# gwall-ceres/HighRes-net

Measured on AMD Instinct MI355X. Metric: SR frames/sec (384x384 out) at B=32, n_views=32, higher is better.
Workload: dtype bf16

## Files before the change

highres-net_amd/hrnet_hip/csrc/conv3x3_v6_impl.h:

```cpp
#pragma once
#include <type_traits>
#include "conv3x3.h"

#ifndef V6_ABL
#define V6_ABL 0
#endif
#ifndef V6_ST_AUX
#define V6_ST_AUX 2
#endif
#ifndef V6_RES_NT
#define V6_RES_NT 1
#endif
#ifndef V6_BAL
#define V6_BAL 4
#endif

#ifdef V6_STAMP
extern __device__ unsigned long long hrn_v6_stamps[256 * 8 * 24];
#define V6_ST(i) do { unsigned long long t_; asm volatile("s_memtime %0\n\ts_waitcnt lgkmcnt(0)" : "=s"(t_) :: "memory"); if (stamp_on) st[i] = t_; } while (0)
#else
#define V6_ST(i) do {} while (0)
#endif

namespace {

constexpr int T6_H = 16, T6_W = 32;
constexpr int HW6 = T6_W + 2;
constexpr int NPIX6 = (T6_H + 2) * HW6;
constexpr int N_IN6 = (NPIX6 * 64 + 1023) / 1024;
constexpr int IN_BYTES6 = N_IN6 * 1024;
constexpr unsigned OOB6 = 0x80000000u;

template <int COUT, bool X3 = false> struct G6 {
    static constexpr int NCB = COUT / 16;
    static constexpr int NQ = NCB / 2;
    static constexpr int TAP_BYTES = COUT * 64;
    static constexpr int WST = 3 * TAP_BYTES;
    static constexpr int W_PIECES = WST / 1024;
    static constexpr int OFF_IN = 2 * WST;
    static constexpr int OFF_BIAS = OFF_IN + 2 * IN_BYTES6;
    static constexpr int ROW = COUT * 2;
    static constexpr int LB = NCB * 2;
    static constexpr int OFF_FIFO = OFF_BIAS + 512;
    static constexpr int FIFO_WAVE = (LB == 16 && !X3) ? 4096 : 0;
    static constexpr int OFF_HOFF = OFF_FIFO + 8 * FIFO_WAVE;
    static constexpr int LDS_BYTES = OFF_HOFF + (X3 ? 8 * 5 * 256 : 0);
};

typedef __attribute__((address_space(3))) void* lds_ptr6;

template <int N> __device__ __forceinline__ void wait_vm6() {
    static_assert(N >= 0 && N <= 63, "vmcnt");
    asm volatile("s_waitcnt vmcnt(%0)" :: "n"(N) : "memory");
}
__device__ __forceinline__ void wait_vm6_rt(int n) {
    switch (n) {
        case 1: wait_vm6<1>(); break;
        case 2: wait_vm6<2>(); break;
        case 3: wait_vm6<3>(); break;
        case 4: wait_vm6<4>(); break;
        case 5: wait_vm6<5>(); break;
        case 6: wait_vm6<6>(); break;
        case 7: wait_vm6<7>(); break;
        case 8: wait_vm6<8>(); break;
        case 9: wait_vm6<9>(); break;
        default: wait_vm6<0>(); break;
    }
}
__device__ __forceinline__ void barrier6() {
    asm volatile("s_waitcnt lgkmcnt(0)" ::: "memory");
    __builtin_amdgcn_s_barrier();
    asm volatile("" ::: "memory");
}
__device__ __forceinline__ int swz6(int row) { return ((row >> 2) & 1) << 1; }

template <int N, int I = 0, class F> __device__ __forceinline__ void static_for6(F&& f) {
    if constexpr (I < N) { f(std::integral_constant<int, I>{}); static_for6<N, I + 1>(f); }
}

template <int CIN, int COUT, int RESM, bool PAIR, bool X3>
__global__ __launch_bounds__(512, 2) void conv3x3_v6_kernel(const ConvParams p) {
    typedef G6<COUT, X3> GEO;
    static_assert(CIN == 128 || (CIN == 64 && !PAIR), "CIN");
    constexpr int NCH = CIN / 32;
    constexpr int NCC = X3 ? 3 * NCH : NCH;
    constexpr int NCB = GEO::NCB, NQ = GEO::NQ, NSTEP = 3 * NQ, WST = GEO::WST, TAP_BYTES = GEO::TAP_BYTES;
    constexpr int OFF_IN = GEO::OFF_IN, ROW = GEO::ROW, LB = GEO::LB;
    typedef typename std::conditional<LB == 16, u32x4, u32x2>::type lane_row_t;
    constexpr bool RES = RESM != 0;
    constexpr int BAL = COUT == 128 ? V6_BAL : 0;
    extern __shared__ __attribute__((aligned(16))) unsigned char smem[];
    float* bias_lds = (float*)(smem + GEO::OFF_BIAS);
    if (p.only_if_nonpos && p.only_if_nonpos[0] > 0.f) return;

    const int tid = threadIdx.x;
    const int lane = tid & 63;
    const int w = __builtin_amdgcn_readfirstlane(tid >> 6);
    const int c15 = lane & 15, q = lane >> 4;
    const int H = p.H, W = p.W;
    const unsigned hw = (unsigned)(H * W);
    const unsigned tiles_x = (W + T6_W - 1) / T6_W;
    const unsigned tiles_y = (H + T6_H - 1) / T6_H;
    const unsigned tiles = tiles_x * tiles_y;
    const unsigned total = tiles * (unsigned)p.M;
    const unsigned G = gridDim.x;
    const unsigned bid = blockIdx.x;
    const unsigned slot0 = (G & 7) == 0 ? (bid & 7) * (G >> 3) + (bid >> 3) : bid;
    if (slot0 >= total) return;
    const int ntl = (int)((total - slot0 + G - 1) / G);
    unsigned cur_m = slot0 / tiles, cur_t = slot0 - cur_m * tiles;
    const unsigned step_m = G / tiles, step_t = G - step_m * tiles;
    constexpr bool in_pair = PAIR;
    constexpr unsigned in_pitch = in_pair ? 128u : (unsigned)(CIN * 2);
    const size_t src_lo = X3 ? (in_pair ? p.stack_lo : p.in_lo) : 0;
    const unsigned char* const src0 = (const unsigned char*)(in_pair ? p.stack : p.in);
    const unsigned img_bytes = hw * in_pitch;

    auto in_bases = [&](unsigned m, size_t& a, size_t& b) __attribute__((always_inline)) {
        if (in_pair) {
            const unsigned bb = m / (unsigned)p.pair_h, i = m - bb * (unsigned)p.pair_h;
            a = ((size_t)bb * p.pair_vs + i) * hw * 128;
            b = ((size_t)bb * p.pair_vs + (p.pair_last - i)) * hw * 128;
        } else {
            a = b = (size_t)m * hw * in_pitch;
        }
    };
    unsigned hoff[5];
    auto tile_offsets = [&](unsigned t) __attribute__((always_inline)) {
        const int ty = t / tiles_x;
        const int y0 = ty * T6_H, x0 = (t - ty * tiles_x) * T6_W;
        int lq = lane;
        asm volatile("" : "+v"(lq));
#pragma unroll
        for (int jj = 0; jj < 5; ++jj) {
            const int pix = (w + 8 * jj) * 16 + (lq >> 2);
            const int lc = (lq & 3) ^ swz6(pix);
            const int py = pix / HW6, px = pix - py * HW6;
            const int gy = y0 - 1 + py, gx = x0 - 1 + px;
            const bool ok = pix < NPIX6 && (unsigned)gy < (unsigned)H && (unsigned)gx < (unsigned)W;
            const unsigned ho = ok ? (unsigned)(gy * W + gx) * in_pitch + (unsigned)(lc * 16) : OOB6;
            if constexpr (X3) *(unsigned*)(smem + GEO::OFF_HOFF + (w * 5 + jj) * 256 + lq * 4) = ho;
            else hoff[jj] = ho;
        }
    };
    auto dma_halo_v = [&](__amdgpu_buffer_rsrc_t rs, int c, int buf, int jj, unsigned voff) __attribute__((always_inline)) {
        const int j = w + 8 * jj;
        if (j < N_IN6) {
            const unsigned soff = in_pair ? (unsigned)((c & 1) * 64) : (unsigned)(c * 64);
            if (!(V6_ABL & 4)) __builtin_amdgcn_raw_ptr_buffer_load_lds(rs, (lds_ptr6)(smem + OFF_IN + buf * IN_BYTES6 + j * 1024), 16, voff, soff, 0, 0);
        }
    };
    auto hoff_lds = [&](int jj) __attribute__((always_inline)) -> unsigned {
        return *(const unsigned*)(smem + GEO::OFF_HOFF + (w * 5 + jj) * 256 + lane * 4);
    };
    auto dma_halo = [&](__amdgpu_buffer_rsrc_t rs, int c, int buf, int jj) __attribute__((always_inline)) {
        if constexpr (X3) dma_halo_v(rs, c, buf, jj, hoff_lds(jj));
        else dma_halo_v(rs, c, buf, jj, hoff[jj]);
    };
    constexpr unsigned W_PLANE = 9u * CIN * COUT * 2u;
    const __amdgpu_buffer_rsrc_t rs_w = __builtin_amdgcn_make_buffer_rsrc((void*)p.wpk, 0, (int)(W_PLANE * (X3 ? 2 : 1)), 0x00020000);
    const unsigned w_lane_off = (unsigned)((lane >> 2) * (NCB * 128) + (((lane & 3) ^ swz6(lane >> 2)) << 4));
    auto dma_w = [&](int c, int tg, int slot_, int t3, unsigned plane_off) __attribute__((always_inline)) {
        const int qq = w + 8 * t3;
        if (qq < GEO::W_PIECES) {
            const int kx = qq / NCB, jb = qq - kx * NCB;
            const unsigned soff = plane_off + (unsigned)(((c >> 1) * 9 + tg * 3 + kx) * (COUT * 128) + (c & 1) * 64 + jb * 128);
            if (!(V6_ABL & 4)) __builtin_amdgcn_raw_ptr_buffer_load_lds(rs_w, (lds_ptr6)(smem + slot_ * WST + kx * TAP_BYTES + jb * 1024), 16, w_lane_off, soff, 0, 0);
        }
    };
    constexpr int NW3 = (GEO::W_PIECES + 7) / 8;
    const int n_in = w < (N_IN6 & 7) ? (N_IN6 >> 3) + 1 : (N_IN6 >> 3);

    const float act_slope = p.slope ? p.slope[0] : 1.f;
    const float act_pick = act_slope <= 1.f ? __builtin_inff() : -__builtin_inff();

    const unsigned lds0 = (unsigned)(__UINTPTR_TYPE__)(__attribute__((address_space(3))) unsigned char*)smem;
    const unsigned a_off = lds0 + (unsigned)(c15 * 64 + ((q ^ swz6(c15)) << 4));
    unsigned baddr[4][3];
#pragma unroll
    for (int j = 0; j < 4; ++j)
#pragma unroll
        for (int kx = 0; kx < 3; ++kx) {
            const int pix = (2 * w + j) * HW6 + c15 + kx;
            baddr[j][kx] = lds0 + (unsigned)OFF_IN + (unsigned)(pix << 6) + ((unsigned)(q << 4) ^ (unsigned)((pix & 4) << 3));
        }

    f32x4 acc[NCB][4];
#ifdef V6_STAMP
    unsigned long long st[24];
#pragma unroll
    for (int i = 0; i < 24; ++i) st[i] = 0;
    bool stamp_on = false;
#endif

    if (tid < COUT) bias_lds[tid] = p.bias[tid];
    size_t inA, inB;
    in_bases(cur_m, inA, inB);
    tile_offsets(cur_t);
    {
        const __amdgpu_buffer_rsrc_t rs = __builtin_amdgcn_make_buffer_rsrc((void*)(src0 + inA), 0, (int)img_bytes, 0x00020000);
#pragma unroll
        for (int t3 = 0; t3 < NW3; ++t3) dma_w(0, 0, 0, t3, 0u);
#pragma unroll
        for (int jj = 0; jj < 5; ++jj) dma_halo(rs, 0, 0, jj);
    }
    wait_vm6<0>();
    barrier6();

    for (int tl = 0; tl < ntl; ++tl) {
        const bool more_tiles = tl + 1 < ntl;
#ifdef V6_STAMP
        stamp_on = false;
        if (RESM == 2 && !PAIR && ntl >= 32 && tl == 1) { stamp_on = true; V6_ST(20); }
        if (RESM == 2 && !PAIR && ntl >= 32 && tl == 2) { stamp_on = true; V6_ST(21); stamp_on = false; }
#endif
        unsigned nxt_t = cur_t + step_t, nxt_m = cur_m + step_m;
        if (nxt_t >= tiles) { nxt_t -= tiles; ++nxt_m; }
        size_t nxA = inA, nxB = inB;
        if (more_tiles) in_bases(nxt_m, nxA, nxB);
#pragma unroll
        for (int cb4 = 0; cb4 < NCB; cb4 += 4) {
            const f32x4 b = *(const f32x4*)(bias_lds + NCB * c15 + cb4);
#pragma unroll
            for (int e = 0; e < 4; ++e)
#pragma unroll
                for (int pxb = 0; pxb < 4; ++pxb) acc[cb4 + e][pxb] = f32x4{b[e], b[e], b[e], b[e]};
        }
        const int ty_ = cur_t / tiles_x;
        const int y0 = ty_ * T6_H, x0 = (cur_t - ty_ * tiles_x) * T6_W;
        const unsigned char *resA = nullptr, *resB = nullptr;
        unsigned char* outp;
        float res_alpha = 1.f;
        {
            size_t oimg = cur_m;
            if (p.out_h > 0) {
                const unsigned ob = cur_m / (unsigned)p.out_h, oi = cur_m - ob * (unsigned)p.out_h;
                oimg = (size_t)ob * p.out_vs + oi;
                if (RESM == 3) {
                    resA = resB = (const unsigned char*)p.res + ((size_t)ob * p.res_vs + oi) * hw * 128;
                    if (p.alphas) res_alpha = p.alphas[(size_t)ob * p.alpha_vs + (p.pair_last - oi)];
                }
            }
            if (RESM == 2) {
                const unsigned bb = cur_m / (unsigned)p.pair_h, i = cur_m - bb * (unsigned)p.pair_h;
                resA = (const unsigned char*)p.stack + ((size_t)bb * p.pair_vs + i) * hw * 128;
                resB = (const unsigned char*)p.stack + ((size_t)bb * p.pair_vs + (p.pair_last - i)) * hw * 128;
            }
            if (RESM == 1) resA = resB = (const unsigned char*)p.res + (size_t)cur_m * hw * ROW;
            outp = (unsigned char*)p.out + oimg * hw * ROW;
        }
        auto res_src = [&](int r, int j) __attribute__((always_inline)) -> const unsigned char* {
            int lq = lane;
            asm volatile("" : "+v"(lq));
            const int c15r = lq & 15, qr = lq >> 4;
            const int gy = y0 + 2 * w + (r >> 1), gyc = gy < H ? gy : H - 1;
            const int gx = x0 + 16 * (r & 1) + 4 * qr + j, gxc = gx < W ? gx : W - 1;
            const unsigned char* view = (RESM == 2 && c15r >= 8) ? resB : resA;
            constexpr int RPITCH = RESM == 1 ? ROW : 128;
            if (V6_ABL & 64) return resA + ((unsigned)(((gyc * W + gxc) & 511) * RPITCH) + (RESM == 2 ? (unsigned)((c15r & 7) * 16) : (unsigned)(c15r * LB)));
            return view + ((unsigned)((gyc * W + gxc) * RPITCH) + (RESM == 2 ? (unsigned)((c15r & 7) * 16) : (unsigned)(c15r * LB)));
        };
        constexpr bool FIFO = RES && LB == 16 && !X3;
        auto res_dma0 = [&]() __attribute__((always_inline)) {
#pragma unroll
            for (int j = 0; j < 4; ++j)
                if (!(V6_ABL & 16))
                    __builtin_amdgcn_global_load_lds((const __attribute__((address_space(1))) void*)res_src(0, j),
                                                     (lds_ptr6)(smem + GEO::OFF_FIFO + w * GEO::FIFO_WAVE + j * 1024), 16, 0, V6_RES_NT ? 2 : 0);
        };

        int c = 0, ps = 0;
        for (int cc = 0; cc < NCC; ++cc) {
            if ((cc > 0 || tl > 0) && (!X3 || ps != 1)) {
                const unsigned d = (X3 ? ps == 2 : (c & 1) != 0) ? (unsigned)IN_BYTES6 : (unsigned)-IN_BYTES6;
#pragma unroll
                for (int j = 0; j < 4; ++j)
#pragma unroll
                    for (int kx = 0; kx < 3; ++kx) baddr[j][kx] += d;
            }
            if (cc == NCC - 1) {
                inA = nxA; inB = nxB;
                if (more_tiles) tile_offsets(nxt_t);
            }
            auto stage = [&](auto tg_c) __attribute__((always_inline)) {
                constexpr int tg = decltype(tg_c)::value;
#ifdef V6_STAMP
                const bool so_ = stamp_on;
                stamp_on = so_ && (cc == 1 || (cc == NCC - 1 && tg == 2));
                const int sb_ = cc == 1 ? 4 * tg : 12;
                V6_ST(sb_ + 0);
#endif
                const int slot_r = (cc + tg) & 1;
                const bool have_next = cc < NCC - 1 || tg < 2 || more_tiles;
                const bool next_chunk = (!X3 || ps != 1) && (cc < NCC - 1 || more_tiles);
                const int tg2 = (tg + 1) % 3;
                int c2 = c;
                unsigned wpl2 = 0;
                if (X3) {
                    int ps2 = ps;
                    if (tg == 2) { if (++ps2 == 3) { ps2 = 0; c2 = (c + 1) & (NCH - 1); } }
                    wpl2 = ps2 == 1 ? W_PLANE : 0u;
                } else {
                    c2 = (c + (tg + 1) / 3) & (NCH - 1);
                }
                const bool nlo = X3 && ps == 0;
                const int cn = nlo ? c : (c + 1) & (NCH - 1);
                const int nbuf = X3 ? (nlo ? 1 : 0) : (cn & 1);
                size_t hb = ((in_pair && cn >= 2) ? inB : inA) + (nlo ? src_lo : (size_t)0);
                if constexpr (X3) {
                    hb = (size_t)(unsigned)__builtin_amdgcn_readfirstlane((int)(unsigned)hb) |
                         ((size_t)(unsigned)__builtin_amdgcn_readfirstlane((int)(unsigned)(hb >> 32)) << 32);
                }
                const __amdgpu_buffer_rsrc_t rs_h = __builtin_amdgcn_make_buffer_rsrc((void*)(src0 + hb), 0, (int)img_bytes, 0x00020000);
                unsigned hst[3] = {0u, 0u, 0u};
                if constexpr (X3) {
                    if (tg < 2 && next_chunk) {
#pragma unroll
                        for (int k = 0; k < (tg == 0 ? 3 : 2); ++k) hst[k] = hoff_lds(tg == 0 ? k : 3 + k);
                        asm volatile("s_waitcnt lgkmcnt(0)" : "+v"(hst[0]), "+v"(hst[1]), "+v"(hst[2]));
                    }
                }
                auto issue_item = [&](int it) __attribute__((always_inline)) {
                    if (it < NW3) { if (have_next) dma_w(c2, tg2, slot_r ^ 1, it, wpl2); }
                    else if (tg == 0 && it < NW3 + 3) {
                        if (next_chunk) { if constexpr (X3) dma_halo_v(rs_h, cn, nbuf, it - NW3, hst[it - NW3]); else dma_halo(rs_h, cn, nbuf, it - NW3); }
                    } else if (tg == 1 && it < NW3 + 2) {
                        if (next_chunk) { if constexpr (X3) dma_halo_v(rs_h, cn, nbuf, it - NW3 + 3, hst[it - NW3]); else dma_halo(rs_h, cn, nbuf, it - NW3 + 3); }
                    }
                };
                constexpr int N_ITEMS = NW3 + (tg == 0 ? 3 : tg == 1 ? 2 : 0);
                static_assert(N_ITEMS <= NSTEP, "one DMA item per step");
                int halo_out = 0;
                if (next_chunk) halo_out = tg == 0 ? 3 : tg == 1 ? n_in - 3 : 0;
                if (FIFO && tg == 2 && cc == NCC - 1 && !(V6_ABL & 2)) res_dma0();
                const unsigned abase = a_off + (unsigned)(slot_r * WST);
                bf16x8 fa[2][2], fb[2][4];
                auto rd = [&](bf16x8& dst, unsigned addr, int imm) __attribute__((always_inline)) {
                    if (V6_ABL & 32) asm volatile("; no read" : "=v"(dst) : "v"(addr), "n"(imm));
                    else asm volatile("ds_read_b128 %0, %1 offset:%2" : "=v"(dst) : "v"(addr), "n"(imm));
                };
                auto load_b1 = [&](int tap, int pxb) __attribute__((always_inline)) {
                    rd(fb[tap & 1][pxb], baddr[(pxb >> 1) + tg][tap], (pxb & 1) * 1024);
                };
                auto load_a1 = [&](int i, int k) __attribute__((always_inline)) {
                    rd(fa[i & 1][k], abase, (i / NQ) * TAP_BYTES + (i % NQ) * 2048 + k * 1024);
                };
                if (BAL && w >= 4) __builtin_amdgcn_s_setprio(1);
#pragma unroll
                for (int pxb = 0; pxb < 4; ++pxb) load_b1(0, pxb);
                load_a1(0, 0);
                load_a1(0, 1);
                __builtin_amdgcn_sched_barrier(0);
                static_for6<NSTEP>([&](auto i_c) __attribute__((always_inline)) {
                    constexpr int i = decltype(i_c)::value;
                    constexpr int qt = i % NQ, tap = i / NQ, bs = tap & 1;
                    constexpr bool a_next = i + 1 < NSTEP;
                    constexpr bool b_cur = qt == (NQ > 1 ? 1 : 0) && tap + 1 < 3;
                    constexpr bool b_prev = i >= 1 && ((i - 1) % NQ) == (NQ > 1 ? 1 : 0) && (i - 1) / NQ + 1 < 3;
                    constexpr int n0 = (b_prev && NQ == 2) ? 0 : 1 + (b_prev ? 4 : 0);
                    constexpr int n4 = (b_prev ? 4 : 0) + (a_next ? 2 : 0) + (b_cur ? 2 : 0);
#pragma unroll
                    for (int g = 0; g < 8; ++g) {
                        const int k = g >> 2, pxb = g & 3;
                        if (g == 0) {
                            if (n0 == 0) asm volatile("s_waitcnt lgkmcnt(0)" : "+v"(fa[i & 1][0]), "+v"(fb[bs][0]), "+v"(fb[bs][1]), "+v"(fb[bs][2]), "+v"(fb[bs][3]));
                            else if (n0 == 1) asm volatile("s_waitcnt lgkmcnt(1)" : "+v"(fa[i & 1][0]), "+v"(fb[bs][0]));
                            else asm volatile("s_waitcnt lgkmcnt(5)" : "+v"(fa[i & 1][0]), "+v"(fb[bs][0]));
                        } else if (g == 4) {
                            if (n4 == 0) asm volatile("s_waitcnt lgkmcnt(0)" : "+v"(fa[i & 1][1]));
                            else if (n4 == 2) asm volatile("s_waitcnt lgkmcnt(2)" : "+v"(fa[i & 1][1]));
                            else if (n4 == 4) asm volatile("s_waitcnt lgkmcnt(4)" : "+v"(fa[i & 1][1]));
                            else if (n4 == 6) asm volatile("s_waitcnt lgkmcnt(6)" : "+v"(fa[i & 1][1]));
                            else asm volatile("s_waitcnt lgkmcnt(8)" : "+v"(fa[i & 1][1]));
                        } else if (k == 0) asm volatile("" : "+v"(fb[bs][pxb]));
                        if (V6_ABL & 1) asm volatile("" : "+v"(acc[qt * 2 + k][pxb]) : "v"(fa[i & 1][k]), "v"(fb[bs][pxb]));
                        else acc[qt * 2 + k][pxb] = __builtin_amdgcn_mfma_f32_16x16x32_bf16(fb[bs][pxb], fa[i & 1][k], acc[qt * 2 + k][pxb], 0, 0, 0);
                        if (g < 2 && a_next) load_a1(i + 1, g);
                        if (g >= 2 && g < 6 && b_cur) load_b1(tap + 1, g - 2);
                        if (g == 7 && i < N_ITEMS) issue_item(i);
                        if (BAL && g == 7 && i == (NSTEP * BAL) / 8 - 1 && w >= 4) __builtin_amdgcn_s_setprio(0);
                        __builtin_amdgcn_sched_barrier(0);
                    }
                });
                V6_ST(sb_ + 1);
                wait_vm6_rt(halo_out);
                V6_ST(sb_ + 2);
                if (tg == 2 && cc == NCC - 1 && (V6_ABL & 2)) {
#pragma unroll
                    for (int cb = 0; cb < NCB; ++cb)
#pragma unroll
                        for (int pxb = 0; pxb < 4; ++pxb) asm volatile("" :: "v"(acc[cb][pxb]));
                }
                if constexpr (X3) {
                if (tg == 2 && cc == NCC - 1 && !(V6_ABL & 2)) {
                    __builtin_amdgcn_s_waitcnt(0x0F70);
                    int le = lane;
                    asm volatile("" : "+v"(le));
                    const int c15e = le & 15, qe = le >> 4;
                    const size_t ob_ = (size_t)outp;
                    unsigned char* const outu = (unsigned char*)((size_t)(unsigned)__builtin_amdgcn_readfirstlane((int)(unsigned)ob_) |
                                                                 ((size_t)(unsigned)__builtin_amdgcn_readfirstlane((int)(unsigned)(ob_ >> 32)) << 32));
                    const __amdgpu_buffer_rsrc_t rs_out = __builtin_amdgcn_make_buffer_rsrc((void*)outu, 0, (int)(hw * ROW), 0x00020000);
                    const __amdgpu_buffer_rsrc_t rs_out_lo = __builtin_amdgcn_make_buffer_rsrc((void*)(outu + p.out_lo), 0, (int)(hw * ROW), 0x00020000);
                    const size_t res_lo_off = RESM == 2 ? p.stack_lo : p.res_lo;
                    lane_row_t rq[8][4];
                    auto res_load = [&](int r, int pl) __attribute__((always_inline)) {
#pragma unroll
                        for (int j = 0; j < 4; ++j)
                            rq[pl * 4 + r][j] = __builtin_nontemporal_load((const lane_row_t*)(res_src(r, j) + (pl ? res_lo_off : (size_t)0)));
                    };
                    if (RES) {
                        res_load(0, 0); res_load(0, 1); res_load(1, 0);
                        if (LB == 8) res_load(1, 1);
                    }
                    __builtin_amdgcn_sched_barrier(0);
#pragma unroll
                    for (int r = 0; r < 4; ++r) {
                        const int gy = y0 + 2 * w + (r >> 1);
#pragma unroll
                        for (int j = 0; j < 4; ++j) {
                            lane_row_t oh, ol;
                            const lane_row_t rh = rq[r][j], rl = rq[4 + r][j];
#pragma unroll
                            for (int i = 0; i < NCB / 2; ++i) {
                                float xa = acc[2 * i][r][j], xb = acc[2 * i + 1][r][j];
                                xa = __builtin_amdgcn_fmed3f(xa, act_slope * xa, act_pick);
                                xb = __builtin_amdgcn_fmed3f(xb, act_slope * xb, act_pick);
                                if (RES) {
                                    const float ra = __uint_as_float(rh[i] << 16), rb = __uint_as_float(rh[i] & 0xffff0000u);
                                    if (RESM == 3) { xa = ra + res_alpha * xa; xb = rb + res_alpha * xb; }
                                    else { xa += ra; xb += rb; }
                                    xa += __uint_as_float(rl[i] << 16); xb += __uint_as_float(rl[i] & 0xffff0000u);
                                }
                                const unsigned h = pack2_bf16(xa, xb);
                                oh[i] = h;
                                ol[i] = pack2_bf16(xa - __uint_as_float(h << 16), xb - __uint_as_float(h & 0xffff0000u));
                            }
                            const int gx = x0 + 16 * (r & 1) + 4 * qe + j;
                            const unsigned voff = ((unsigned)(gy * W + gx) * (unsigned)ROW + (unsigned)(c15e * LB)) | ((unsigned)(W - 1 - gx) & OOB6) | (gy < H ? 0u : OOB6);
                            if constexpr (LB == 16) {
                                __builtin_amdgcn_raw_buffer_store_b128(oh, rs_out, voff, 0, V6_ST_AUX);
                                __builtin_amdgcn_raw_buffer_store_b128(ol, rs_out_lo, voff, 0, V6_ST_AUX);
                            } else {
                                __builtin_amdgcn_raw_buffer_store_b64(oh, rs_out, voff, 0, V6_ST_AUX);
                                __builtin_amdgcn_raw_buffer_store_b64(ol, rs_out_lo, voff, 0, V6_ST_AUX);
                            }
                        }
                        if (RES) {
                            __builtin_amdgcn_sched_barrier(0);
                            if (LB == 16) {
                                if (r == 0) { res_load(1, 1); res_load(2, 0); res_load(2, 1); }
                                if (r == 1) { res_load(3, 0); res_load(3, 1); }
                            } else if (r < 2) { res_load(r + 2, 0); res_load(r + 2, 1); }
                        }
                        __builtin_amdgcn_sched_barrier(0);
                    }
                }
                } else
                if (tg == 2 && cc == NCC - 1 && !(V6_ABL & 2)) {
                    __builtin_amdgcn_s_waitcnt(0x0F70);
                    int le = lane;
                    asm volatile("" : "+v"(le));
                    const int c15e = le & 15, qe = le >> 4;
                    const __amdgpu_buffer_rsrc_t rs_out = __builtin_amdgcn_make_buffer_rsrc((void*)outp, 0, (int)(hw * ROW), 0x00020000);
                    lane_row_t rq[4][4];
                    auto res_load = [&](int r) __attribute__((always_inline)) {
#pragma unroll
                        for (int j = 0; j < 4; ++j) {
                            if (V6_ABL & 16) { rq[r][j] = lane_row_t{}; rq[r][j][0] = (unsigned)le; }
#if V6_RES_NT
                            else rq[r][j] = __builtin_nontemporal_load((const lane_row_t*)res_src(r, j));
#else
                            else rq[r][j] = *(const lane_row_t*)res_src(r, j);
#endif
                        }
                    };
                    if (RES) {
                        if (FIFO) {
                            res_load(1); res_load(2);
#pragma unroll
                            for (int j = 0; j < 4; ++j) rq[0][j] = *(const lane_row_t*)(smem + GEO::OFF_FIFO + w * GEO::FIFO_WAVE + j * 1024 + le * 16);
                        } else { res_load(0); res_load(1); }
                    }
                    __builtin_amdgcn_sched_barrier(0);
                    {
#pragma unroll
                        for (int r = 0; r < 4; ++r) {
                            const int gy = y0 + 2 * w + (r >> 1);
#pragma unroll
                            for (int j = 0; j < 4; ++j) {
                                lane_row_t o;
                                const lane_row_t rv = rq[r][j];
#pragma unroll
                                for (int i = 0; i < NCB / 2; ++i) {
                                    float xa = acc[2 * i][r][j], xb = acc[2 * i + 1][r][j];
                                    xa = __builtin_amdgcn_fmed3f(xa, act_slope * xa, act_pick);
                                    xb = __builtin_amdgcn_fmed3f(xb, act_slope * xb, act_pick);
                                    if (RES) {
                                        const float ra = __uint_as_float(rv[i] << 16), rb = __uint_as_float(rv[i] & 0xffff0000u);
                                        if (RESM == 3) { xa = ra + res_alpha * xa; xb = rb + res_alpha * xb; }
                                        else { xa += ra; xb += rb; }
                                    }
                                    o[i] = pack2_bf16(xa, xb);
                                }
                                const int gx = x0 + 16 * (r & 1) + 4 * qe + j;
                                const unsigned voff = ((unsigned)(gy * W + gx) * (unsigned)ROW + (unsigned)(c15e * LB)) | ((unsigned)(W - 1 - gx) & OOB6) | (gy < H ? 0u : OOB6);
                                if (V6_ABL & 8) asm volatile("" :: "v"(o), "v"(voff));
                                else if constexpr (LB == 16) __builtin_amdgcn_raw_buffer_store_b128(o, rs_out, voff, 0, V6_ST_AUX);
                                else __builtin_amdgcn_raw_buffer_store_b64(o, rs_out, voff, 0, V6_ST_AUX);
                            }
                            if (RES && (FIFO ? r == 0 : r < 2)) res_load(FIFO ? 3 : r + 2);
                            __builtin_amdgcn_sched_barrier(0);
                        }
                    }
                }
#ifdef V6_STAMP
                if (cc == NCC - 1 && tg == 2) V6_ST(16);
#endif
                barrier6();
                V6_ST(sb_ + 3);
#ifdef V6_STAMP
                stamp_on = so_;
#endif
            };
            stage(std::integral_constant<int, 0>{});
            stage(std::integral_constant<int, 1>{});
            stage(std::integral_constant<int, 2>{});
            if (X3) { if (++ps == 3) { ps = 0; ++c; } } else ++c;
        }
        cur_m = nxt_m; cur_t = nxt_t;
    }
    wait_vm6<0>();
#ifdef V6_STAMP
    if (RESM == 2 && !PAIR && ntl >= 32 && lane == 0) {
#pragma unroll
        for (int i = 0; i < 24; ++i) hrn_v6_stamps[(bid * 8 + w) * 24 + i] = st[i];
    }
#endif
}

template <int CIN, int COUT, int RESM, bool PAIR, bool X3>
int launch_v6(const ConvParams& p, long grid, hipStream_t stream) {
    typedef G6<COUT, X3> GEO;
    static_assert(GEO::LDS_BYTES <= 160 * 1024, "LDS budget");
    { const int rc_lds = hrn_allow_lds((const void*)conv3x3_v6_kernel<CIN, COUT, RESM, PAIR, X3>, GEO::LDS_BYTES); if (rc_lds) return rc_lds; }
    hipLaunchKernelGGL((conv3x3_v6_kernel<CIN, COUT, RESM, PAIR, X3>), dim3((unsigned)grid), dim3(512), GEO::LDS_BYTES, stream, p);
    HRN_LAUNCH_CHECK();
    return 0;
}

}

#define V6_COMMON_ROWS(ROW)                   \
    ROW(64, 128, 0, false, "64x128")          \
    ROW(128, 128, 0, true, "128x128")         \
    ROW(128, 128, 2, true, "128x128+res")     \
    ROW(128, 128, 0, false, "128x128")        \
    ROW(128, 128, 1, false, "128x128+res")    \
    ROW(128, 128, 2, false, "128x128+res")    \
    ROW(128, 64, 0, false, "128x64")          \
    ROW(128, 64, 3, false, "128x64+res")
```

Baseline: 2072.

## Merge two X3 passes into one wide pass for 64-channel conv

For the three-pass (X3) conv with 64 output channels, two of the three passes are merged into one "wide" pass. That pass loads weights from both planes together and runs twice as many MFMA column steps against a single halo load. This cuts the pass count from three to two per input chunk, so halo reloads, barriers and stage overhead drop by about a third. The cost is a larger weight LDS slot and more complex schedule logic, now split out into a helper header.

```diff
diff --git a/highres-net_amd/hrnet_hip/csrc/conv3x3_v6_impl.h b/highres-net_amd/hrnet_hip/csrc/conv3x3_v6_impl.h
--- a/highres-net_amd/hrnet_hip/csrc/conv3x3_v6_impl.h
+++ b/highres-net_amd/hrnet_hip/csrc/conv3x3_v6_impl.h
@@ -1,6 +1,7 @@
 #pragma once
 #include <type_traits>
 #include "conv3x3.h"
+#include "v6_schedule.h"
 
 #ifndef V6_ABL
 #define V6_ABL 0
@@ -13,6 +14,13 @@
 #endif
 #ifndef V6_BAL
 #define V6_BAL 4
+#endif
+
+#ifndef V6_BAL_WIDE
+#define V6_BAL_WIDE 4
+#endif
+#ifndef V6_WIDE
+#define V6_WIDE 1
 #endif
 
 #ifdef V6_STAMP
@@ -32,9 +40,12 @@
 constexpr unsigned OOB6 = 0x80000000u;
 
 template <int COUT, bool X3 = false> struct G6 {
+    static constexpr bool WIDE = X3 && COUT == 64 && V6_WIDE;
+    static constexpr V6Walk WALK = WIDE ? V6_X3_WIDE : X3 ? V6_X3_THREE : V6_PLAIN;
     static constexpr int NCB = COUT / 16;
     static constexpr int NQ = NCB / 2;
-    static constexpr int TAP_BYTES = COUT * 64;
+    static constexpr int NWB = WIDE ? 2 * NCB : NCB;
+    static constexpr int TAP_BYTES = NWB * 1024;
     static constexpr int WST = 3 * TAP_BYTES;
     static constexpr int W_PIECES = WST / 1024;
     static constexpr int OFF_IN = 2 * WST;
@@ -83,12 +94,14 @@
     typedef G6<COUT, X3> GEO;
     static_assert(CIN == 128 || (CIN == 64 && !PAIR), "CIN");
     constexpr int NCH = CIN / 32;
-    constexpr int NCC = X3 ? 3 * NCH : NCH;
-    constexpr int NCB = GEO::NCB, NQ = GEO::NQ, NSTEP = 3 * NQ, WST = GEO::WST, TAP_BYTES = GEO::TAP_BYTES;
+    constexpr V6Walk WALK = GEO::WALK;
+    constexpr bool WIDE = GEO::WIDE;
+    constexpr int NCC = v6_passes(WALK) * NCH;
+    constexpr int NCB = GEO::NCB, NQ = GEO::NQ, WST = GEO::WST, TAP_BYTES = GEO::TAP_BYTES;
     constexpr int OFF_IN = GEO::OFF_IN, ROW = GEO::ROW, LB = GEO::LB;
     typedef typename std::conditional<LB == 16, u32x4, u32x2>::type lane_row_t;
     constexpr bool RES = RESM != 0;
-    constexpr int BAL = COUT == 128 ? V6_BAL : 0;
+    constexpr int BAL128 = COUT == 128 ? V6_BAL : 0;
     extern __shared__ __attribute__((aligned(16))) unsigned char smem[];
     float* bias_lds = (float*)(smem + GEO::OFF_BIAS);
     if (p.only_if_nonpos && p.only_if_nonpos[0] > 0.f) return;
@@ -160,11 +173,14 @@
     constexpr unsigned W_PLANE = 9u * CIN * COUT * 2u;
     const __amdgpu_buffer_rsrc_t rs_w = __builtin_amdgcn_make_buffer_rsrc((void*)p.wpk, 0, (int)(W_PLANE * (X3 ? 2 : 1)), 0x00020000);
     const unsigned w_lane_off = (unsigned)((lane >> 2) * (NCB * 128) + (((lane & 3) ^ swz6(lane >> 2)) << 4));
-    auto dma_w = [&](int c, int tg, int slot_, int t3, unsigned plane_off) __attribute__((always_inline)) {
+    auto dma_w = [&](int c, int tg, int slot_, int t3, unsigned plane_off, bool both) __attribute__((always_inline)) {
         const int qq = w + 8 * t3;
-        if (qq < GEO::W_PIECES) {
-            const int kx = qq / NCB, jb = qq - kx * NCB;
-            const unsigned soff = plane_off + (unsigned)(((c >> 1) * 9 + tg * 3 + kx) * (COUT * 128) + (c & 1) * 64 + jb * 128);
+        const int nwb = both ? GEO::NWB : NCB;
+        if (qq < 3 * nwb) {
+            const int kx = qq / nwb, jb = qq - kx * nwb;
+            const int cbk = both ? (jb & (NCB - 1)) : jb;
+            if (both) plane_off = jb >= NCB ? W_PLANE : 0u;
+            const unsigned soff = plane_off + (unsigned)(((c >> 1) * 9 + tg * 3 + kx) * (COUT * 128) + (c & 1) * 64 + cbk * 128);
             if (!(V6_ABL & 4)) __builtin_amdgcn_raw_ptr_buffer_load_lds(rs_w, (lds_ptr6)(smem + slot_ * WST + kx * TAP_BYTES + jb * 1024), 16, w_lane_off, soff, 0, 0);
         }
     };
@@ -200,7 +216,7 @@
     {
         const __amdgpu_buffer_rsrc_t rs = __builtin_amdgcn_make_buffer_rsrc((void*)(src0 + inA), 0, (int)img_bytes, 0x00020000);
 #pragma unroll
-        for (int t3 = 0; t3 < NW3; ++t3) dma_w(0, 0, 0, t3, 0u);
+        for (int t3 = 0; t3 < NW3; ++t3) dma_w(0, 0, 0, t3, 0u, WIDE);
 #pragma unroll
         for (int jj = 0; jj < 5; ++jj) dma_halo(rs, 0, 0, jj);
     }
@@ -271,8 +287,8 @@
 
         int c = 0, ps = 0;
         for (int cc = 0; cc < NCC; ++cc) {
-            if ((cc > 0 || tl > 0) && (!X3 || ps != 1)) {
-                const unsigned d = (X3 ? ps == 2 : (c & 1) != 0) ? (unsigned)IN_BYTES6 : (unsigned)-IN_BYTES6;
+            if ((cc > 0 || tl > 0) && (WALK != V6_X3_THREE || ps != 1)) {
+                const unsigned d = v6_halo_buffer(WALK, c, ps) != 0 ? (unsigned)IN_BYTES6 : (unsigned)-IN_BYTES6;
 #pragma unroll
                 for (int j = 0; j < 4; ++j)
 #pragma unroll
@@ -282,30 +298,28 @@
                 inA = nxA; inB = nxB;
                 if (more_tiles) tile_offsets(nxt_t);
             }
-            auto stage = [&](auto tg_c) __attribute__((always_inline)) {
+            auto stage = [&](auto tg_c, auto wd_c) __attribute__((always_inline)) {
                 constexpr int tg = decltype(tg_c)::value;
+                constexpr bool WD = decltype(wd_c)::value;
+                static_assert(!WD || WIDE, "wide stage");
+                constexpr int NQS = WD ? 2 * NQ : NQ, NSTEP = 3 * NQS;
+                constexpr bool WD2 = WIDE && (tg < 2 ? WD : !WD);
+                constexpr int BAL = WD ? V6_BAL_WIDE : BAL128;
+                constexpr int NW3N = WIDE ? (WD2 ? 3 : 2) : NW3;
 #ifdef V6_STAMP
                 const bool so_ = stamp_on;
                 stamp_on = so_ && (cc == 1 || (cc == NCC - 1 && tg == 2));
                 const int sb_ = cc == 1 ? 4 * tg : 12;
                 V6_ST(sb_ + 0);
 #endif
-                const int slot_r = (cc + tg) & 1;
+                const int slot_r = v6_slot_read(cc, tg);
                 const bool have_next = cc < NCC - 1 || tg < 2 || more_tiles;
-                const bool next_chunk = (!X3 || ps != 1) && (cc < NCC - 1 || more_tiles);
-                const int tg2 = (tg + 1) % 3;
-                int c2 = c;
-                unsigned wpl2 = 0;
-                if (X3) {
-                    int ps2 = ps;
-                    if (tg == 2) { if (++ps2 == 3) { ps2 = 0; c2 = (c + 1) & (NCH - 1); } }
-                    wpl2 = ps2 == 1 ? W_PLANE : 0u;
-                } else {
-                    c2 = (c + (tg + 1) / 3) & (NCH - 1);
-                }
-                const bool nlo = X3 && ps == 0;
-                const int cn = nlo ? c : (c + 1) & (NCH - 1);
-                const int nbuf = X3 ? (nlo ? 1 : 0) : (cn & 1);
+                const bool next_chunk = v6_fetches<WALK>(ps) && (cc < NCC - 1 || more_tiles);
+                const int tg2 = v6_next_tap_row(tg), c2 = v6_next_chunk<WALK, NCH, tg>(c, ps);
+                const unsigned wpl2 = v6_w_planes(WALK, v6_next_pass<WALK, tg>(ps)) == V6_W_LO ? W_PLANE : 0u;
+                const bool nlo = v6_fetch_lo<WALK>(ps);
+                const int cn = v6_fetch_chunk<WALK, NCH>(c, ps);
+                const int nbuf = v6_halo_fill<WALK>(cn, nlo);
                 size_t hb = ((in_pair && cn >= 2) ? inB : inA) + (nlo ? src_lo : (size_t)0);
                 if constexpr (X3) {
                     hb = (size_t)(unsigned)__builtin_amdgcn_readfirstlane((int)(unsigned)hb) |
@@ -321,14 +335,14 @@
                     }
                 }
                 auto issue_item = [&](int it) __attribute__((always_inline)) {
-                    if (it < NW3) { if (have_next) dma_w(c2, tg2, slot_r ^ 1, it, wpl2); }
-                    else if (tg == 0 && it < NW3 + 3) {
-                        if (next_chunk) { if constexpr (X3) dma_halo_v(rs_h, cn, nbuf, it - NW3, hst[it - NW3]); else dma_halo(rs_h, cn, nbuf, it - NW3); }
-                    } else if (tg == 1 && it < NW3 + 2) {
-                        if (next_chunk) { if constexpr (X3) dma_halo_v(rs_h, cn, nbuf, it - NW3 + 3, hst[it - NW3]); else dma_halo(rs_h, cn, nbuf, it - NW3 + 3); }
+                    if (it < NW3N) { if (have_next) dma_w(c2, tg2, slot_r ^ 1, it, wpl2, WD2); }
+                    else if (tg == 0 && it < NW3N + 3) {
+                        if (next_chunk) { if constexpr (X3) dma_halo_v(rs_h, cn, nbuf, it - NW3N, hst[it - NW3N]); else dma_halo(rs_h, cn, nbuf, it - NW3N); }
+                    } else if (tg == 1 && it < NW3N + 2) {
+                        if (next_chunk) { if constexpr (X3) dma_halo_v(rs_h, cn, nbuf, it - NW3N + 3, hst[it - NW3N]); else dma_halo(rs_h, cn, nbuf, it - NW3N + 3); }
                     }
                 };
-                constexpr int N_ITEMS = NW3 + (tg == 0 ? 3 : tg == 1 ? 2 : 0);
+                constexpr int N_ITEMS = NW3N + (tg == 0 ? 3 : tg == 1 ? 2 : 0);
                 static_assert(N_ITEMS <= NSTEP, "one DMA item per step");
                 int halo_out = 0;
                 if (next_chunk) halo_out = tg == 0 ? 3 : tg == 1 ? n_in - 3 : 0;
@@ -343,7 +357,7 @@
                     rd(fb[tap & 1][pxb], baddr[(pxb >> 1) + tg][tap], (pxb & 1) * 1024);
                 };
                 auto load_a1 = [&](int i, int k) __attribute__((always_inline)) {
-                    rd(fa[i & 1][k], abase, (i / NQ) * TAP_BYTES + (i % NQ) * 2048 + k * 1024);
+                    rd(fa[i & 1][k], abase, (i / NQS) * TAP_BYTES + (i % NQS) * 2048 + k * 1024);
                 };
                 if (BAL && w >= 4) __builtin_amdgcn_s_setprio(1);
 #pragma unroll
@@ -353,11 +367,11 @@
                 __builtin_amdgcn_sched_barrier(0);
                 static_for6<NSTEP>([&](auto i_c) __attribute__((always_inline)) {
                     constexpr int i = decltype(i_c)::value;
-                    constexpr int qt = i % NQ, tap = i / NQ, bs = tap & 1;
+                    constexpr int qt = i % NQS, tap = i / NQS, bs = tap & 1;
                     constexpr bool a_next = i + 1 < NSTEP;
-                    constexpr bool b_cur = qt == (NQ > 1 ? 1 : 0) && tap + 1 < 3;
-                    constexpr bool b_prev = i >= 1 && ((i - 1) % NQ) == (NQ > 1 ? 1 : 0) && (i - 1) / NQ + 1 < 3;
-                    constexpr int n0 = (b_prev && NQ == 2) ? 0 : 1 + (b_prev ? 4 : 0);
+                    constexpr bool b_cur = qt == (NQS > 1 ? 1 : 0) && tap + 1 < 3;
+                    constexpr bool b_prev = i >= 1 && ((i - 1) % NQS) == (NQS > 1 ? 1 : 0) && (i - 1) / NQS + 1 < 3;
+                    constexpr int n0 = (b_prev && NQS == 2) ? 0 : 1 + (b_prev ? 4 : 0);
                     constexpr int n4 = (b_prev ? 4 : 0) + (a_next ? 2 : 0) + (b_cur ? 2 : 0);
 #pragma unroll
                     for (int g = 0; g < 8; ++g) {
@@ -373,8 +387,9 @@
                             else if (n4 == 6) asm volatile("s_waitcnt lgkmcnt(6)" : "+v"(fa[i & 1][1]));
                             else asm volatile("s_waitcnt lgkmcnt(8)" : "+v"(fa[i & 1][1]));
                         } else if (k == 0) asm volatile("" : "+v"(fb[bs][pxb]));
-                        if (V6_ABL & 1) asm volatile("" : "+v"(acc[qt * 2 + k][pxb]) : "v"(fa[i & 1][k]), "v"(fb[bs][pxb]));
-                        else acc[qt * 2 + k][pxb] = __builtin_amdgcn_mfma_f32_16x16x32_bf16(fb[bs][pxb], fa[i & 1][k], acc[qt * 2 + k][pxb], 0, 0, 0);
+                        const int cb = (qt * 2 + k) & (NCB - 1);
+                        if (V6_ABL & 1) asm volatile("" : "+v"(acc[cb][pxb]) : "v"(fa[i & 1][k]), "v"(fb[bs][pxb]));
+                        else acc[cb][pxb] = __builtin_amdgcn_mfma_f32_16x16x32_bf16(fb[bs][pxb], fa[i & 1][k], acc[cb][pxb], 0, 0, 0);
                         if (g < 2 && a_next) load_a1(i + 1, g);
                         if (g >= 2 && g < 6 && b_cur) load_b1(tap + 1, g - 2);
                         if (g == 7 && i < N_ITEMS) issue_item(i);
@@ -385,14 +400,14 @@
                 V6_ST(sb_ + 1);
                 wait_vm6_rt(halo_out);
                 V6_ST(sb_ + 2);
-                if (tg == 2 && cc == NCC - 1 && (V6_ABL & 2)) {
+                if (!WD && tg == 2 && cc == NCC - 1 && (V6_ABL & 2)) {
 #pragma unroll
                     for (int cb = 0; cb < NCB; ++cb)
 #pragma unroll
                         for (int pxb = 0; pxb < 4; ++pxb) asm volatile("" :: "v"(acc[cb][pxb]));
                 }
                 if constexpr (X3) {
-                if (tg == 2 && cc == NCC - 1 && !(V6_ABL & 2)) {
+                if (!WD && tg == 2 && cc == NCC - 1 && !(V6_ABL & 2)) {
                     __builtin_amdgcn_s_waitcnt(0x0F70);
                     int le = lane;
                     asm volatile("" : "+v"(le));
@@ -523,10 +538,18 @@
                 stamp_on = so_;
 #endif
             };
-            stage(std::integral_constant<int, 0>{});
-            stage(std::integral_constant<int, 1>{});
-            stage(std::integral_constant<int, 2>{});
-            if (X3) { if (++ps == 3) { ps = 0; ++c; } } else ++c;
+            if (WIDE && ps == 0) {
+                if constexpr (WIDE) {
+                    stage(std::integral_constant<int, 0>{}, std::true_type{});
+                    stage(std::integral_constant<int, 1>{}, std::true_type{});
+                    stage(std::integral_constant<int, 2>{}, std::true_type{});
+                }
+            } else {
+                stage(std::integral_constant<int, 0>{}, std::false_type{});
+                stage(std::integral_constant<int, 1>{}, std::false_type{});
+                stage(std::integral_constant<int, 2>{}, std::false_type{});
+            }
+            v6_advance(WALK, c, ps);
         }
         cur_m = nxt_m; cur_t = nxt_t;
     }
diff --git a/highres-net_amd/hrnet_hip/csrc/v6_schedule.h b/highres-net_amd/hrnet_hip/csrc/v6_schedule.h
--- /dev/null
+++ b/highres-net_amd/hrnet_hip/csrc/v6_schedule.h
@@ -0,0 +1,78 @@
+#pragma once
+
+#if defined(__HIPCC__)
+#define V6S_FN __host__ __device__ __forceinline__ constexpr
+#else
+#define V6S_FN inline constexpr
+#endif
+
+enum V6Walk { V6_PLAIN = 0, V6_X3_THREE = 1, V6_X3_WIDE = 2 };
+enum { V6_W_HI = 1, V6_W_LO = 2 };
+
+
+V6S_FN int v6_passes(V6Walk walk) { return walk == V6_X3_THREE ? 3 : walk == V6_X3_WIDE ? 2 : 1; }
+
+V6S_FN int v6_x_plane(V6Walk walk, int ps) { return walk == V6_X3_THREE ? ps == 2 : walk == V6_X3_WIDE ? ps == 1 : 0; }
+V6S_FN int v6_halo_buffer(V6Walk walk, int c, int ps) { return walk == V6_PLAIN ? (c & 1) : v6_x_plane(walk, ps); }
+template <V6Walk walk> V6S_FN bool v6_changes_buffer(int ps) {
+    if constexpr (walk != V6_X3_THREE) return true;
+    else return ps != 1;
+}
+template <V6Walk walk> V6S_FN bool v6_fetches(int ps) {
+    if constexpr (walk != V6_X3_THREE) return true;
+    else return ps != 1;
+}
+V6S_FN int v6_w_planes(V6Walk walk, int ps) {
+    return walk == V6_X3_THREE ? (ps == 1 ? V6_W_LO : V6_W_HI) : walk == V6_X3_WIDE ? (ps == 0 ? V6_W_HI | V6_W_LO : V6_W_HI) : V6_W_HI;
+}
+
+V6S_FN int v6_slot_read(int cc, int tg) { return (cc + tg) & 1; }
+template <int tg> V6S_FN bool v6_has_next(bool pass_follows, bool more_tiles) { return pass_follows || tg < 2 || more_tiles; }
+template <V6Walk walk> V6S_FN bool v6_fetch(int ps, bool pass_follows, bool more_tiles) {
+    return v6_fetches<walk>(ps) && (pass_follows || more_tiles);
+}
+template <V6Walk walk> V6S_FN bool v6_fetch_lo(int ps) { return walk != V6_PLAIN && ps == 0; }
+template <V6Walk walk, int nch> V6S_FN int v6_fetch_chunk(int c, int ps) { return v6_fetch_lo<walk>(ps) ? c : (c + 1) & (nch - 1); }
+template <V6Walk walk> V6S_FN int v6_halo_fill(int fetch_chunk, bool fetch_lo) { return walk != V6_PLAIN ? (fetch_lo ? 1 : 0) : (fetch_chunk & 1); }
+V6S_FN int v6_next_tap_row(int tg) { return (tg + 1) % 3; }
+template <V6Walk walk, int tg> V6S_FN int v6_next_pass(int ps) { return tg < 2 ? ps : ps + 1 == v6_passes(walk) ? 0 : ps + 1; }
+template <V6Walk walk, int nch, int tg> V6S_FN int v6_next_chunk(int c, int ps) {
+    if (walk == V6_PLAIN) return (c + (tg + 1) / 3) & (nch - 1);
+    int c2 = c, ps2 = ps;
+    if (tg == 2) { if (++ps2 == v6_passes(walk)) { ps2 = 0; c2 = (c + 1) & (nch - 1); } }
+    return c2;
+}
+
+struct V6Stage {
+    int chunk, pass, tap_row;
+    int x_plane, w_planes;
+    int slot_read, slot_fill;
+    int halo_read, halo_fill;
+    int fetch_chunk, fetch_plane;
+    int next_chunk, next_pass, next_tap_row, next_w_planes;
+};
+
+template <V6Walk walk, int nch, int tg> V6S_FN V6Stage v6_stage(int cc, int c, int ps, bool more_tiles) {
+    V6Stage s = {};
+    s.chunk = c; s.pass = ps; s.tap_row = tg;
+    s.x_plane = v6_x_plane(walk, ps);
+    s.w_planes = v6_w_planes(walk, ps);
+    s.slot_read = v6_slot_read(cc, tg);
+    const bool pass_follows = cc < v6_passes(walk) * nch - 1;
+    s.slot_fill = v6_has_next<tg>(pass_follows, more_tiles) ? s.slot_read ^ 1 : -1;
+    s.halo_read = v6_halo_buffer(walk, c, ps);
+    const bool fetch = tg < 2 && v6_fetch<walk>(ps, pass_follows, more_tiles);
+    s.halo_fill = fetch ? v6_halo_fill<walk>(v6_fetch_chunk<walk, nch>(c, ps), v6_fetch_lo<walk>(ps)) : -1;
+    s.fetch_chunk = fetch ? v6_fetch_chunk<walk, nch>(c, ps) : -1;
+    s.fetch_plane = fetch ? (int)v6_fetch_lo<walk>(ps) : -1;
+    s.next_tap_row = v6_next_tap_row(tg);
+    s.next_pass = v6_next_pass<walk, tg>(ps);
+    s.next_chunk = v6_next_chunk<walk, nch, tg>(c, ps);
+    s.next_w_planes = v6_w_planes(walk, s.next_pass);
+    return s;
+}
+
+V6S_FN void v6_advance(V6Walk walk, int& c, int& ps) {
+    if (walk == V6_PLAIN) ++c;
+    else if (++ps == v6_passes(walk)) { ps = 0; ++c; }
+}
```

Result: no change. 2072, median of 3 (-0.0%).
